# WU-CVGL/CasualHDRSplat

Hardware: AMD Instinct MI355X
Metric: train-step images/sec (fwd+bwd raster) @ 1M Gaussians 1080p (higher is better)
Workload: dtype f32; 1 GPU; c3: 1000000 Gaussians, 1920x1080, SH degree 3, HDR radiance + CRF tone-map, 1 pose(s)/view, 1 view(s)/step (one per GPU); num_rendered_R=6777809, R_prime=3025699, pixel_pair_evals_E=559372855, seed=0, binning=sync-free fixed capacity 1.25*R, launch=eager (one enqueue per kernel)

## Files before the change

### casualhdrsplat_amd/csrc/render.hip

```cpp
#include "hs_common.h"

namespace hs {

namespace {

constexpr float kAlphaMin = 1.0f / 255.0f;
constexpr float kAlphaMax = 0.99f;
constexpr float kTmin = 0.0001f;
constexpr float kLogEps = 1e-8f;


enum {
    kStBwdTrips = 0,
    kStBwdEmpty = 1,
    kStBwdActivePix = 2,
    kStBwdCulled = 3,
    kStBwdHist = 4,
    kStBwdStaged = 10,
    kStBwdBatches = 11,
    kStFwdTrips = 12, kStFwdEmpty = 13, kStFwdActivePix = 14, kStFwdCulled = 15, kStFwdStaged = 16, kStFwdBatches = 17,
    kStCount = 24
};
struct WaveStats {
    unsigned long long v[kStCount];
// ... 473 lines not shown
    float sumH = 0.f, sumL = 0.f;
    const float* planes = pose_hdr + (int64_t)f * N * 3 * HW + j;
    for (int k = 0; k < N; ++k) {
        const float Hv = planes[(int64_t)k * 3 * HW];
        sumH += Hv;
        if (hdr && !(flags & HS_FLAG_BLUR_HDR)) sumL += crf_eval(crf, ch, Hv);
    }
    const float inv = 1.f / (float)N;
    const float meanH = sumH * inv;
    pose_hdr[((int64_t)F * N + f) * 3 * HW + j] = meanH;
    if (hdr) {
        if (out_hdr) out_hdr[i] = meanH;
        out_color[i] = (flags & HS_FLAG_BLUR_HDR) ? crf_eval(crf, ch, meanH) : sumL * inv;
    } else {
        out_color[i] = meanH;
    }
}

__global__ void __launch_bounds__(1024) order_tiles_kernel(int nb, int gx, int n_static, const uint32_t* work,
                                                           uint32_t* order) {
    constexpr int kBins = 1024, kT = 1024;
    __shared__ uint32_t s_hist[kBins];
    __shared__ uint32_t s_scan[kT / 64];
    __shared__ uint32_t s_thr_bin, s_thr_take;
    const int x = blockIdx.x, t = threadIdx.x;
    const int per = nb / 8, rem = nb % 8;
    const int cnt = per + (x < rem ? 1 : 0);
    const int n_keep = n_static > x ? (n_static - x + 7) / 8 : 0;
    const int n_light = cnt - n_keep;
    int q_base = 0;
    for (int y = 0; y < x; ++y) q_base += (per + (y < rem ? 1 : 0)) - (n_static > y ? (n_static - y + 7) / 8 : 0);
    const int E = (cnt + kT - 1) / kT;
    const int k0 = t * E, k1 = min(cnt, (t + 1) * E);
    if (E > 64) {
        for (int k = k0; k < k1; ++k) order[x + 8 * k] = (uint32_t)xcd_strip_tile(x + 8 * k, nb, gx);
        return;
    }
    auto block_excl_scan = [&](uint32_t v, uint32_t* total) -> uint32_t {
        uint32_t incl = v;
#pragma unroll
        for (int d = 1; d < 64; d <<= 1) { const uint32_t u = __shfl_up(incl, d); if ((t & 63) >= d) incl += u; }
        __syncthreads();
        if ((t & 63) == 63) s_scan[t >> 6] = incl;
        __syncthreads();
        uint32_t add = 0, tot = 0;
        for (int w = 0; w < kT / 64; ++w) { const uint32_t c = s_scan[w]; if (w < (t >> 6)) add += c; tot += c; }
        *total = tot;
        return add + incl - v;
    };
    auto bin_of = [&](int k) { return (int)min((uint32_t)(kBins - 1), work[xcd_strip_tile(x + 8 * k, nb, gx)] >> 1); };
    s_hist[t] = 0;
    if (t == 0) { s_thr_bin = 0; s_thr_take = 0; }
    __syncthreads();
    for (int k = k0; k < k1; ++k) atomicAdd(&s_hist[bin_of(k)], 1u);
    __syncthreads();
    {
        uint32_t tot;
        const uint32_t h = s_hist[t];
        const uint32_t below = block_excl_scan(h, &tot);
        if (below < (uint32_t)n_light && below + h >= (uint32_t)n_light) { s_thr_bin = t; s_thr_take = (uint32_t)n_light - below; }
    }
    __syncthreads();
    const int thr = (int)s_thr_bin;
    const uint32_t take = s_thr_take;
    uint32_t in_thr = 0;
    for (int k = k0; k < k1; ++k) in_thr += bin_of(k) == thr ? 1u : 0u;
    uint32_t tot_thr;
    uint32_t thr_rank = block_excl_scan(in_thr, &tot_thr);
    uint64_t light_mask = 0;
    uint32_t kept = 0;
    for (int k = k0; k < k1; ++k) {
        const int b = bin_of(k);
        const bool light = n_light > 0 && (b < thr || (b == thr && thr_rank++ < take));
        light_mask |= (uint64_t)light << (k - k0);
        kept += !light;
    }
    uint32_t tot_kept;
    uint32_t kpos = block_excl_scan(kept, &tot_kept);
    uint32_t qpos = (uint32_t)k0 - kpos;
    for (int k = k0; k < k1; ++k) {
        const uint32_t vt = (uint32_t)xcd_strip_tile(x + 8 * k, nb, gx);
        if ((light_mask >> (k - k0)) & 1ull) order[n_static + q_base + (int)qpos++] = vt;
        else order[x + 8 * (int)kpos++] = vt;
    }
}

constexpr int kCrfPixPerWave = 1024;

struct CrfGradArgs {
    int64_t HW; int N, F, flags;
    const float* pose_hdr; Crf crf; const float* exposure; const float* dL_dcolor; float* partials;
    int bx, planes;
};

template <int NW, int NH = 1>
__device__ __forceinline__ void crf_grad_body(const CrfGradArgs& A, const int bxi, const int plane_in,
                                              unsigned long long* const s_tab64) {
    static_assert(NH == 1 || NW == 1, "pieces in turn: one-wave workgroups only");
    constexpr int NP = NW * NH;
    static_assert(NP == 2 || NP == 4, "the pieces' float sums are added in a stated order");
    const int64_t HW = A.HW; const int N = A.N, flags = A.flags; const float* pose_hdr = A.pose_hdr; Crf crf = A.crf;
    const float* exposure = A.exposure; const float* dL_dcolor = A.dL_dcolor; float* partials = A.partials;
    int* const s_tab32 = reinterpret_cast<int*>(s_tab64);
    __shared__ float s_wave[NP][4];
    __shared__ float s_max[NW];
    const int K = crf.K;
    for (int i = threadIdx.x; i < K - 1; i += NW * 64) s_tab64[i] = 0ull;
    const bool blur_hdr = (flags & HS_FLAG_BLUR_HDR) && N > 1;
    const float gs = blur_hdr ? 1.f : 1.f / (float)N;
    const float scale = (float)(K - 1) / (crf.umax - crf.umin);
    const int plane = plane_in;
    const int pose = plane / 3, ch = plane - 3 * pose;
    const int frame = blur_hdr ? pose : (A.F > 1 ? pose / N : 0);
    crf.dt = exposure[frame];
    const float* Hp = pose_hdr + ((int64_t)(blur_hdr ? A.F * N + frame : pose) * 3 + ch) * HW;
    const float* gp = dL_dcolor + ((int64_t)frame * 3 + ch) * HW;
    const float* t = crf.table + ch * K;
    const int lane = threadIdx.x & 63, wave = threadIdx.x >> 6;

    float Hv[NH][16], g[NH][16];
#pragma unroll
    for (int h = 0; h < NH; ++h) {
        const int64_t i16 = ((int64_t)bxi * (NP * 64) + h * 64 + threadIdx.x) * 16;
        if (i16 + 16 <= HW && (HW & 3) == 0) {
#pragma unroll
            for (int q = 0; q < 4; ++q) {
                const float4 h4 = reinterpret_cast<const float4*>(Hp + i16)[q];
                const float4 g4 = reinterpret_cast<const float4*>(gp + i16)[q];
                Hv[h][4 * q] = h4.x; Hv[h][4 * q + 1] = h4.y; Hv[h][4 * q + 2] = h4.z; Hv[h][4 * q + 3] = h4.w;
                g[h][4 * q] = g4.x * gs; g[h][4 * q + 1] = g4.y * gs; g[h][4 * q + 2] = g4.z * gs; g[h][4 * q + 3] = g4.w * gs;
            }
        } else {
#pragma unroll
            for (int e = 0; e < 16; ++e) {
                const bool ok = i16 + e < HW;
                Hv[h][e] = ok ? Hp[i16 + e] : 0.f;
                g[h][e] = ok ? gp[i16 + e] * gs : 0.f;
            }
        }
    }
    float mx = 0.f;
#pragma unroll
    for (int h = 0; h < NH; ++h)
#pragma unroll
        for (int e = 0; e < 16; ++e) mx = fmaxf(mx, fabsf(g[h][e]));
#pragma unroll
    for (int d = 32; d >= 1; d >>= 1) mx = fmaxf(mx, __shfl_xor(mx, d));
    if (lane == 0) s_max[wave] = mx;
    __syncthreads();
    mx = s_max[0];
    if constexpr (NW >= 2) mx = fmaxf(mx, s_max[1 % NW]);
    if constexpr (NW == 4) mx = fmaxf(mx, fmaxf(s_max[2 % NW], s_max[3 % NW]));
    int xexp = 0;
    if (mx > 0.f && mx < 3.0e38f) (void)frexpf(mx, &xexp);
    const float to_fix = ldexpf(1.f, 19 - xexp), from_fix = ldexpf(1.f, xexp - 19);

#pragma unroll
    for (int h = 0; h < NH; ++h) {
        float gexp = 0.f, g_lo = 0.f, g_hi = 0.f;
        int run = -1;
        float r0 = 0.f, r1 = 0.f;
        auto flush = [&]() {
            atomicAdd(&s_tab32[2 * run], __float2int_rn(r0 * to_fix));
            atomicAdd(&s_tab32[2 * run + 1], __float2int_rn(r1 * to_fix));
        };
#pragma unroll
        for (int e = 0; e < 16; ++e) {
            int idx; float f, xv; bool in;
            crf_locate(crf, Hv[h][e], idx, f, xv, in);
            const bool lo = idx == 0 && f == 0.f, hi = idx == K - 2 && f == 1.f;
            g_lo += lo ? g[h][e] : 0.f;
            g_hi += hi ? g[h][e] : 0.f;
            if (!lo && !hi) {
                if (idx != run) {
                    if (run >= 0) flush();
                    run = idx; r0 = 0.f; r1 = 0.f;
                }
                r0 += (1.f - f) * g[h][e];
                r1 += f * g[h][e];
            }
            if (in) gexp += g[h][e] * (t[idx + 1] - t[idx]) * scale * __builtin_amdgcn_rcpf(xv) * Hv[h][e];
        }
        if (run >= 0) flush();
        gexp = wave_sum_hi(gexp);
        g_lo = wave_sum_hi(g_lo);
        g_hi = wave_sum_hi(g_hi);
        if (lane == 63) { s_wave[wave + h][0] = gexp; s_wave[wave + h][1] = g_lo; s_wave[wave + h][2] = g_hi; }
    }
    __syncthreads();
    auto pieces = [&](int c) {
        float v = s_wave[0][c] + s_wave[1][c];
        if constexpr (NP == 4) v = (v + s_wave[2 % NP][c]) + s_wave[3 % NP][c];
        return v;
    };
    float* dst = partials + ((int64_t)plane_in * A.bx + bxi) * (K + 1);
    for (int k = threadIdx.x; k <= K; k += NW * 64) {
        float v;
        if (k == K) {
            v = pieces(0);
        } else {
            long long acc = 0;
            if (k < K - 1) acc += (long long)s_tab32[2 * k];
            if (k > 0) acc += (long long)s_tab32[2 * (k - 1) + 1];
            v = (float)acc * from_fix;
            if (k == 0) v += pieces(1);
            if (k == K - 1) v += pieces(2);
        }
        dst[k] = v;
    }
}

struct RenderBwd {
    int W, H, gx, gy, ntiles, N, F, flags;
    const uint2* ranges; const uint32_t* point_list; const float4* rec; const float* bg;
    const float* final_T; const uint32_t* n_contrib; const float* pose_hdr;
    const float* dL_dcolor; const float* dL_dhdr; const float* dL_dalpha; const float* dL_dinvdepth;
    float4* pair_grads;
    uint8_t* pair_flags;
    const uint8_t* pair_act;
    Crf crf;
    const float* exposure;
    unsigned long long* stats;
    unsigned long long* timeline;
    uint32_t* queue;
    const uint32_t* tile_order;
    int grid_tiles;
    CrfGradArgs crf_tail;
};

__device__ __forceinline__ float pixel_grad(const RenderBwd& p, const Crf& c, int pose, int frame, int ch, int64_t pix, int64_t HW) {
    const float invN = 1.f / (float)p.N;
    const int64_t gpl = ((int64_t)frame * 3 + ch) * HW + pix;
    float g = p.dL_dcolor[gpl];
    if (!(p.flags & HS_FLAG_HDR)) return g * invN;
    float out = 0.f;
    if (p.N == 1 || !(p.flags & HS_FLAG_BLUR_HDR)) {
        const float Hv = p.pose_hdr[((int64_t)pose * 3 + ch) * HW + pix];
        out = crf_grad_H(c, ch, Hv, g * invN);
    } else {
        const float Hm = p.pose_hdr[((int64_t)(p.F * p.N + frame) * 3 + ch) * HW + pix];
        out = crf_grad_H(c, ch, Hm, g) * invN;
    }
    if (p.dL_dhdr) out += p.dL_dhdr[gpl] * invN;
    return out;
}

struct PixB {
    float T, dL0, dL1, dL2, q;
    float dLd;
    uint32_t last;
};

__device__ __forceinline__ void load_pixel_bwd(const RenderBwd& p, PixB& s, bool inside, int pose, int frame, int px, int py) {
    const int64_t HW = (int64_t)p.H * p.W;
    const int64_t pix = (int64_t)py * p.W + px;
    s.T = 0.f; s.dL0 = s.dL1 = s.dL2 = 0.f; s.last = 0;
    if (inside) {
        s.T = p.final_T[(int64_t)pose * HW + pix];
        s.last = p.n_contrib[(int64_t)pose * HW + pix];
        Crf c = p.crf;
        if (p.flags & HS_FLAG_HDR) c.dt = p.exposure[frame];
        s.dL0 = pixel_grad(p, c, pose, frame, 0, pix, HW);
        s.dL1 = pixel_grad(p, c, pose, frame, 1, pix, HW);
        s.dL2 = pixel_grad(p, c, pose, frame, 2, pix, HW);
    }
    float bg_dot = (p.bg[0] * s.dL0 + p.bg[1] * s.dL1) + p.bg[2] * s.dL2;
    if (p.dL_dalpha && inside) bg_dot -= p.dL_dalpha[pix] / (float)p.N;
    s.q = bg_dot;
    s.dLd = (p.dL_dinvdepth && inside) ? p.dL_dinvdepth[pix] / (float)p.N : 0.f;
}

struct PairB {
    f2 T, q, dL0, dL1, dL2, dLd;
};
__device__ __forceinline__ f2 splat(float v) { f2 r = {v, v}; return r; }
__device__ __forceinline__ PairB pack_pair(const PixB& a, const PixB& b) {
    PairB s;
    s.T = f2{a.T, b.T}; s.q = f2{a.q, b.q};
    s.dL0 = f2{a.dL0, b.dL0}; s.dL1 = f2{a.dL1, b.dL1}; s.dL2 = f2{a.dL2, b.dL2};
    s.dLd = f2{a.dLd, b.dLd};
    return s;
}
template <bool DEPTH>
__device__ __forceinline__ void step_bwd_pair(PairB& s, bool act0, bool act1, f2 G, f2 alpha, float o, float r, float g,
                                              float b, float invd, f2& sw, f2& dop, f2& dch) {
    const f2 ae = {act0 ? alpha.x : 0.f, act1 ? alpha.y : 0.f};
    const f2 one_m = splat(1.f) - ae;
    const f2 rcp = {__builtin_amdgcn_rcpf(one_m.x), __builtin_amdgcn_rcpf(one_m.y)};
    s.T *= rcp;
    dch = ae * s.T;
    f2 cd = (splat(r) * s.dL0 + pk_mul_hi(f2{r, g}, s.dL1)) + splat(b) * s.dL2;
    if constexpr (DEPTH) cd += splat(invd) * s.dLd;
    const f2 diff = cd - s.q;
    const f2 gd = G * (diff * s.T);
    s.q += ae * diff;
    dop = f2{act0 ? gd.x : 0.f, act1 ? gd.y : 0.f};
    sw = splat(o) * dop;
}

constexpr int kTailPct = 8;
constexpr int kAccF = 12;
constexpr int kBwdWave = 64;
#ifndef HS_TUNE_BWD_KB
#define HS_TUNE_BWD_KB 48
#endif
#ifndef HS_TUNE_BWD_WAVES
#define HS_TUNE_BWD_WAVES 4
#endif
constexpr int kBwdKB = HS_TUNE_BWD_KB;
constexpr int bwd_stage_floats(int ent_f) { return (kBwdKB + 1) * ent_f > 7 * 256 ? (kBwdKB + 1) * ent_f : 7 * 256; }

__device__ __forceinline__ void lane_pixels4(int lane, int sx, int sy, int& px, int& py0) {
    const int blk = lane >> 4;
    px = sx + 8 * (blk & 1) + (lane & 7);
    py0 = sy + 8 * (blk >> 1) + 4 * ((lane >> 3) & 1);
}

template <bool DEPTH, bool STATS>
__global__ void __launch_bounds__(kBwdWave) __attribute__((amdgpu_waves_per_eu((DEPTH || STATS) ? 1 : HS_TUNE_BWD_WAVES)))
render_bwd_kernel(RenderBwd p) {
    constexpr int KB = kBwdKB;
    constexpr int NV = DEPTH ? 10 : 9;
    constexpr int kEntF = kAccF + 4 * NV;
    constexpr int kEntB = kEntF * 4;
    static_assert(kEntB % 16 == 0, "LDS entry records must stay 16-byte aligned");
    static_assert(KB <= kBwdWave, "one staged entry per lane, one ballot per list");
    constexpr int kSentinel = KB * kEntB;
    constexpr int kListLen = KB + 8;
    constexpr int kStageF = bwd_stage_floats(kEntF);
    __shared__ __attribute__((aligned(16))) float s_ent[kStageF];
    __shared__ uint16_t s_list[4][kListLen];

    const int lane = threadIdx.x;
    if constexpr (!STATS) {
        if ((int)blockIdx.x >= p.grid_tiles) {
            const int qd = (int)blockIdx.x - p.grid_tiles;
            crf_grad_body<1, 2>(p.crf_tail, qd % p.crf_tail.bx, qd / p.crf_tail.bx, reinterpret_cast<unsigned long long*>(s_ent));
            return;
        }
    }
    const int n_tail = (int)((int64_t)p.grid_tiles * kTailPct / 100);
    const int n_static = p.grid_tiles - n_tail;
    for (;;) {
    int bidx = blockIdx.x;
    if ((int)blockIdx.x >= n_static) {
        uint32_t q = 0;
        if (lane == 0) {
            q = atomicAdd(p.queue, 1u);
            if (q == 2u * (uint32_t)n_tail - 1u) atomicExch(p.queue, 0u);
        }
        q = __builtin_amdgcn_readfirstlane(q);
        if (q >= (uint32_t)n_tail) return;
        bidx = n_static + (int)q;
    }
    const int vt = p.tile_order ? (int)p.tile_order[bidx] : xcd_strip_tile(bidx, p.grid_tiles, p.gx);
    const int pose = vt / p.ntiles;
    const int tile = vt - pose * p.ntiles;
    const int tx = tile % p.gx, ty = tile / p.gx;
    const int blk = lane >> 4;
    const int plane = 2 * (blk & 1) + (blk >> 1);
    const int sx = tx * kTile, sy = ty * kTile;
    int px, py0;
    lane_pixels4(lane, sx, sy, px, py0);
    const float pxf = (float)px;
    const f2 pyfA = {(float)py0, (float)(py0 + 1)}, pyfB = {(float)(py0 + 2), (float)(py0 + 3)};

    unsigned long long t_start = 0;
    if constexpr (STATS) t_start = wall_clock64();
    const uint2 range = p.ranges[vt];

    PairB psA, psB;
    uint32_t last0, last1, last2, last3;
    {
        __syncthreads();
        const int qc = lane & 15, qr = lane >> 4;
        const int frame = p.F > 1 ? pose / p.N : 0;
        float* const o = s_ent;
#pragma unroll
        for (int k = 0; k < 4; ++k) {
            const int row = qr + 4 * k;
            PixB t;
            load_pixel_bwd(p, t, sx + qc < p.W && sy + row < p.H, pose, frame, sx + qc, sy + row);
            const int r = row * 16 + qc;
            o[r] = t.T; o[256 + r] = t.dL0; o[512 + r] = t.dL1; o[768 + r] = t.dL2; o[1024 + r] = t.q;
            o[1280 + r] = t.dLd; o[1536 + r] = __uint_as_float(t.last);
        }
        __syncthreads();
        const float* const m = o + (py0 - sy) * 16 + (px - sx);
        psA.T = f2{m[0], m[16]};                  psB.T = f2{m[32], m[48]};
        psA.dL0 = f2{m[256], m[256 + 16]};        psB.dL0 = f2{m[256 + 32], m[256 + 48]};
        psA.dL1 = f2{m[512], m[512 + 16]};        psB.dL1 = f2{m[512 + 32], m[512 + 48]};
        psA.dL2 = f2{m[768], m[768 + 16]};        psB.dL2 = f2{m[768 + 32], m[768 + 48]};
        psA.q = f2{m[1024], m[1024 + 16]};        psB.q = f2{m[1024 + 32], m[1024 + 48]};
        psA.dLd = f2{m[1280], m[1280 + 16]};      psB.dLd = f2{m[1280 + 32], m[1280 + 48]};
        last0 = __float_as_uint(m[1536]); last1 = __float_as_uint(m[1536 + 16]);
        last2 = __float_as_uint(m[1536 + 32]); last3 = __float_as_uint(m[1536 + 48]);
        __syncthreads();
        if (lane < kAccF) s_ent[KB * kEntF + lane] = 0.f;
    }

    const int n_proc = (int)__builtin_amdgcn_readfirstlane(wave_max_u32(max(max(last0, last1), max(last2, last3))));

    int red_off = -1;
    const int red_j = lane & 3;
    {
        const int k = (lane & 15) >> 2;
        if (red_j == 0) red_off = k;
        else if (red_j == 1) red_off = 4 + k;
        else if (red_j == 2 && k == 0) red_off = 8;
        else if (DEPTH && red_j == 2 && k == 1) red_off = 9;
        if (red_off >= 0) red_off = (kAccF + NV * plane + red_off) * 4;
    }
    char* const ent = reinterpret_cast<char*>(s_ent);
    float* const my_ent = s_ent + lane * kEntF;
    const uint16_t* const my_list = s_list[blk];
    WaveStats ws;
    if constexpr (STATS) ws.clear();
    const int nb = (n_proc + KB - 1) / KB;
    uint32_t id_next = 0, act_next = 0;
    if (nb > 0) {
        const int base = (nb - 1) * KB;
        if (lane < n_proc - base) {
            id_next = p.point_list[range.x + base + lane];
            act_next = p.pair_act[(int64_t)range.x + base + lane];
        }
    }
    for (int bi = nb - 1; bi >= 0; --bi) {
        const int base = bi * KB;
        const int cnt = min(KB, n_proc - base);
        if constexpr (STATS) { ws.v[kStBwdStaged] += cnt; ws.v[kStBwdBatches] += 1; }
        __syncthreads();
        const uint32_t act = lane < cnt ? act_next : 0u;
        const bool taken = act != 0;
        if (taken) {
            const float4* r = p.rec + kRecF4 * (int64_t)id_next;
            float4 ra = r[0], rb = r[1];
            float4 rc = r[2];
            if constexpr (DEPTH) rc.y = 1.f / rc.y;
            scale_entry(ra, rb);
            reinterpret_cast<float4*>(my_ent)[0] = ra;
            reinterpret_cast<float4*>(my_ent)[1] = rb;
            reinterpret_cast<float4*>(my_ent)[2] = rc;
        }
        if (bi > 0 && lane < KB) {
            id_next = p.point_list[range.x + base - KB + lane];
            act_next = p.pair_act[(int64_t)range.x + base - KB + lane];
        }
        {
            int maxn = 0;
            [[maybe_unused]] int n_half[2] = {0, 0};
#pragma unroll
            for (int b = 0; b < 4; ++b) {
                const uint32_t gbit = 1u << (2 * (b & 1) + (b >> 1));
                uint16_t* lst = s_list[b];
                const uint64_t m = __ballot((act & gbit) != 0);
                const int c = __popcll(m);
                if ((m >> lane) & 1ull) lst[c - 1 - mask_prefix(m)] = (uint16_t)(lane * kEntB);
#pragma unroll
                for (int t = lane; t < kListLen; t += 64)
                    if (t >= c) lst[t] = (uint16_t)kSentinel;
                maxn = max(maxn, c);
                n_half[b >> 1] = max(n_half[b >> 1], c);
            }
            if constexpr (STATS) ws.v[kStBwdCulled] += (uint32_t)cnt - (uint32_t)__popcll(__ballot(taken));
            __syncthreads();
            const int lim0 = ((int)last0 - base) * kEntB, lim1 = ((int)last1 - base) * kEntB;
            const int lim2 = ((int)last2 - base) * kEntB, lim3 = ((int)last3 - base) * kEntB;
            int jb = (int)my_list[0];
            const int n_it = __builtin_amdgcn_readfirstlane(maxn);
            for (int ti = 0; ti < n_it; ++ti) {
                int jn = (int)my_list[ti + 1];
                asm("" : "+v"(jn));
                const float4 a = *reinterpret_cast<const float4*>(ent + jb);
                const float4 b = *reinterpret_cast<const float4*>(ent + jb + 16);
                const float2 c = *reinterpret_cast<const float2*>(ent + jb + 32);
                const float cb = c.x;
                const float invd = DEPTH ? c.y : 0.f;
                const float dx = a.x - pxf;
                const f2 dyA = a.y - pyfA, dyB = a.y - pyfB;
                const float t = a.z * dx * dx, u = a.w * dx;
                const f2 pwA = dyA * (b.x * dyA + u) + t, pwB = dyB * (b.x * dyB + u) + t;
                const float G0 = hs_exp2(pwA.x), G1 = hs_exp2(pwA.y), G2 = hs_exp2(pwB.x), G3 = hs_exp2(pwB.y);
                const float al0 = fminf(kAlphaMax, b.y * G0), al1 = fminf(kAlphaMax, b.y * G1);
                const float al2 = fminf(kAlphaMax, b.y * G2), al3 = fminf(kAlphaMax, b.y * G3);
                const bool act0 = (jb < lim0) && (pwA.x <= 0.f) && (al0 >= kAlphaMin);
                const bool act1 = (jb < lim1) && (pwA.y <= 0.f) && (al1 >= kAlphaMin);
                const bool act2 = (jb < lim2) && (pwB.x <= 0.f) && (al2 >= kAlphaMin);
                const bool act3 = (jb < lim3) && (pwB.y <= 0.f) && (al3 >= kAlphaMin);
                if constexpr (STATS) {
                    const uint64_t lanes = __ballot(act0 || act1 || act2 || act3);
#pragma unroll
                    for (int h = 0; h < 2; ++h) {
                        if (ti < n_half[h]) {
                            const int nl = __popc((uint32_t)(lanes >> (32 * h)));
                            ws.v[kStBwdTrips] += 1;
                            ws.v[kStBwdEmpty] += nl == 0;
                            const int bin = nl == 0 ? 0 : nl <= 4 ? 1 : nl <= 8 ? 2 : nl <= 16 ? 3 : nl <= 32 ? 4 : 5;
                            ws.v[kStBwdHist + bin] += 1;
                        }
                    }
                    ws.v[kStBwdActivePix] += __popcll(__ballot(act0)) + __popcll(__ballot(act1)) + __popcll(__ballot(act2)) +
                                             __popcll(__ballot(act3));
                }
                f2 swA, dopA, dchA, swB, dopB, dchB;
                step_bwd_pair<DEPTH>(psA, act0, act1, f2{G0, G1}, f2{al0, al1}, b.y, b.z, b.w, cb, invd, swA, dopA, dchA);
                step_bwd_pair<DEPTH>(psB, act2, act3, f2{G2, G3}, f2{al2, al3}, b.y, b.z, b.w, cb, invd, swB, dopB, dchB);
                const f2 sw = swA + swB;
                const f2 mA = swA * dyA, mB = swB * dyB;
                const f2 m = mA + mB;
                const f2 m2 = mA * dyA + mB * dyB;
                const f2 c0 = dchA * psA.dL0 + dchB * psB.dL0;
                const f2 c1 = dchA * psA.dL1 + dchB * psB.dL1;
                const f2 c2 = dchA * psA.dL2 + dchB * psB.dL2;
                float g[9];
                g[0] = (sw.x + sw.y) * dx;
                g[1] = m.x + m.y;
                g[2] = g[0] * dx;
                g[3] = g[1] * dx;
                g[4] = m2.x + m2.y;
                g[5] = (dopA.x + dopA.y) + (dopB.x + dopB.y);
                g[6] = c0.x + c0.y;
                g[7] = c1.x + c1.y;
                g[8] = c2.x + c2.y;
                float g9 = 0.f;
                if constexpr (DEPTH) {
                    const f2 cd = dchA * psA.dLd + dchB * psB.dLd;
                    g9 = cd.x + cd.y;
                }
                float t0, t1, t2;
                row_reduce<DEPTH>(g, g9, t0, t1, t2);
                if (red_off >= 0) *reinterpret_cast<float*>(ent + jb + red_off) = red_j == 0 ? t0 : red_j == 1 ? t1 : t2;
                jb = jn;
            }
        }
        __syncthreads();
        if (taken) {
            float v[10] = {0.f, 0.f, 0.f, 0.f, 0.f, 0.f, 0.f, 0.f, 0.f, 0.f};
#pragma unroll
            for (int pl = 0; pl < 4; ++pl) {
                const bool on = (act >> pl) & 1u;
#pragma unroll
                for (int q = 0; q < NV; ++q) {
                    const float x = my_ent[kAccF + NV * pl + q];
                    v[q] += on ? x : 0.f;
                }
            }
            const float4 a = reinterpret_cast<const float4*>(my_ent)[0];
            const float4 c = reinterpret_cast<const float4*>(my_ent)[2];
            const float A = a.z * (-2.f / kLog2e), B = a.w * (-1.f / kLog2e), C = my_ent[4] * (-2.f / kLog2e);
            const float ddelx_dx = 0.5f * (float)p.W, ddely_dy = 0.5f * (float)p.H;
            const float gmx = -(A * v[0] + B * v[1]) * ddelx_dx;
            const float gmy = -(C * v[1] + B * v[0]) * ddely_dy;
            const int rad = __float_as_int(c.z);
            const uint32_t off = __float_as_uint(c.w);
            const int rminx = min(p.gx, max(0, (int)((a.x - (float)rad) / (float)kTile)));
            const int rminy = min(p.gy, max(0, (int)((a.y - (float)rad) / (float)kTile)));
            const int rmaxx = min(p.gx, max(0, (int)((a.x + (float)rad + (float)(kTile - 1)) / (float)kTile)));
            const int64_t slot = (int64_t)off + (int64_t)(ty - rminy) * (rmaxx - rminx) + (tx - rminx);
            p.pair_flags[slot] = 1;
            float4* o = p.pair_grads + kPairF4 * slot;
            o[0] = make_float4(gmx, gmy, -0.5f * v[2], -v[3]);
            o[1] = make_float4(-0.5f * v[4], v[5], v[6], v[7]);
            float zero = 0.f;
            asm volatile("" : "+v"(zero));
            o[2] = make_float4(v[8], v[9], zero, zero);
            if constexpr (kPairF4 == 4) o[3] = make_float4(zero, zero, zero, zero);
        }
    }
    if constexpr (STATS) {
        ws.flush(p.stats);
        if (p.timeline && lane == 0) {
            p.timeline[3 * bidx + 0] = t_start;
            p.timeline[3 * bidx + 1] = wall_clock64();
            const uint32_t xcc = __builtin_amdgcn_s_getreg((3 << 11) | (0 << 6) | 20);
            const uint32_t hw = __builtin_amdgcn_s_getreg((31 << 11) | (0 << 6) | 4);
            p.timeline[3 * bidx + 2] = ((unsigned long long)xcc << 32) | hw;
        }
    }
    if ((int)blockIdx.x < n_static) return;
    }
}

__global__ void __launch_bounds__(256) crf_grad_kernel(CrfGradArgs A) {
    extern __shared__ unsigned long long s_crf_tab[];
    crf_grad_body<4>(A, (int)blockIdx.x, (int)blockIdx.y, s_crf_tab);
}

__global__ void __launch_bounds__(256) crf_reduce_kernel(CrfReduce c) { crf_reduce_block(c, (int)blockIdx.x); }

}

static bool orders_tiles(int grid) { return grid <= 6 * 3072; }


int launch_render_fwd(const hs_fwd_args& a, const hs_layout& L, hipStream_t s, unsigned long long* stats) {
    const hs_dims& d = a.dims;
    RenderFwd p;
    p.W = d.W; p.H = d.H; p.gx = (d.W + kTile - 1) / kTile;
    const int gy = (d.H + kTile - 1) / kTile;
    const int F = frames_of(d);
    p.ntiles = p.gx * gy; p.N = d.n_poses / F; p.flags = a.flags;
    char* bin = (char*)a.binning; char* img = (char*)a.image; char* geom = (char*)a.geom;
    p.ranges = (const uint2*)(bin + L.ranges); p.point_list = (const uint32_t*)(bin + L.point_list);
    p.rec = (const float4*)(geom + L.rec); p.bg = a.bg;
    p.out_color = a.out_color; p.out_hdr = a.out_hdr;
    p.final_T = (float*)(img + L.final_T); p.n_contrib = (uint32_t*)(img + L.n_contrib);
    const bool need_pose = (a.flags & HS_FLAG_HDR) || p.N > 1;
    p.pose_hdr = need_pose ? (float*)(img + L.pose_hdr) : nullptr;
    p.crf.table = a.crf_table; p.crf.K = a.crf_K; p.crf.umin = a.crf_umin; p.crf.umax = a.crf_umax; p.crf.dt = 1.f;
    p.exposure = a.exposure;
    p.out_invdepth = a.out_invdepth;
    p.stats = stats; p.timeline = nullptr;
    p.pair_act = (uint8_t*)bin + L.pair_act;
    p.tile_work = (uint32_t*)(img + L.tile_work);
    const int grid = p.ntiles * d.n_poses;
    if (stats) {
        if (a.out_invdepth) render_fwd_kernel<true, true><<<grid, kBatch, 0, s>>>(p);
        else render_fwd_kernel<false, true><<<grid, kBatch, 0, s>>>(p);
    } else if (a.out_invdepth) render_fwd_kernel<true, false><<<grid, kBatch, 0, s>>>(p);
    else render_fwd_kernel<false, false><<<grid, kBatch, 0, s>>>(p);
    HS_LAUNCH_CHECK();
    if (orders_tiles(grid)) {
        const int n_static = grid - (int)((int64_t)grid * kTailPct / 100);
        order_tiles_kernel<<<8, 1024, 0, s>>>(grid, p.gx, n_static, p.tile_work, (uint32_t*)(img + L.tile_order));
        HS_LAUNCH_CHECK();
    }
    if (p.N > 1) {
        const int64_t HW = (int64_t)d.W * d.H;
        resolve_kernel<<<ceil_div((int64_t)F * 3 * HW, 256), 256, 0, s>>>(HW, p.N, F, a.flags, p.pose_hdr, p.crf, a.exposure,
                                                                         a.out_color, a.out_hdr);
        HS_LAUNCH_CHECK();
    }
    return HS_OK;
}

static bool crf_grad_args(const hs_bwd_args& a, const hs_layout& L, CrfGradArgs& A, int waves = 4) {
    const hs_dims& d = a.dims;
    if (!((a.flags & HS_FLAG_HDR) && (a.dL_dcrf_table || a.dL_dexposure))) return false;
    A.crf.table = a.crf_table; A.crf.K = a.crf_K; A.crf.umin = a.crf_umin; A.crf.umax = a.crf_umax; A.crf.dt = 1.f;
    A.HW = (int64_t)d.W * d.H; A.F = frames_of(d); A.N = d.n_poses / A.F; A.flags = a.flags;
    A.partials = (float*)((char*)a.bwd + L.crf_partials);
    A.pose_hdr = (const float*)((const char*)a.image + L.pose_hdr);
    A.exposure = a.exposure; A.dL_dcolor = a.dL_dout_color;
    const bool blur_hdr = (a.flags & HS_FLAG_BLUR_HDR) && A.N > 1;
    A.planes = 3 * (blur_hdr ? A.F : d.n_poses);
    A.bx = ceil_div(A.HW, (int64_t)waves * kCrfPixPerWave);
    return true;
}

int launch_crf_bwd(const hs_bwd_args& a, const hs_layout& L, hipStream_t s, CrfReduce* defer, bool in_render_tail) {
    CrfGradArgs A;
    if (!crf_grad_args(a, L, A, in_render_tail ? 2 : 4)) return HS_OK;
    if (!in_render_tail)
        crf_grad_kernel<<<dim3(A.bx, A.planes), 256, (size_t)(a.crf_K - 1) * sizeof(unsigned long long), s>>>(A);
    CrfReduce cr;
    cr.partials = A.partials; cr.bx = A.bx; cr.planes = A.planes; cr.K = a.crf_K; cr.d_table = a.dL_dcrf_table;
    cr.F = A.F;
    cr.d_exposure = a.dL_dexposure; cr.nblocks = ceil_div(3 * a.crf_K + cr.F, 4);
    if (defer) *defer = cr;
    else crf_reduce_kernel<<<cr.nblocks, 256, 0, s>>>(cr);
    HS_LAUNCH_CHECK();
    return HS_OK;
}

int launch_render_bwd(const hs_bwd_args& a, const hs_layout& L, hipStream_t s, unsigned long long* stats,
                      unsigned long long* timeline, bool crf_in_tail) {
    const hs_dims& d = a.dims;
    RenderBwd p;
    p.W = d.W; p.H = d.H; p.gx = (d.W + kTile - 1) / kTile; p.gy = (d.H + kTile - 1) / kTile;
    p.F = frames_of(d);
    p.ntiles = p.gx * p.gy; p.N = d.n_poses / p.F; p.flags = a.flags;
    const char* bin = (const char*)a.binning; const char* img = (const char*)a.image; const char* geom = (const char*)a.geom;
    p.ranges = (const uint2*)(bin + L.ranges); p.point_list = (const uint32_t*)(bin + L.point_list);
    p.rec = (const float4*)(geom + L.rec); p.bg = a.bg;
    p.final_T = (const float*)(img + L.final_T); p.n_contrib = (const uint32_t*)(img + L.n_contrib);
    p.pose_hdr = (const float*)(img + L.pose_hdr);
    p.dL_dcolor = a.dL_dout_color; p.dL_dhdr = a.dL_dout_hdr; p.dL_dalpha = a.dL_dout_alpha;
    p.dL_dinvdepth = a.dL_dout_invdepth;
    p.pair_grads = (float4*)((char*)a.bwd + L.pair_grads);
    p.crf.table = a.crf_table; p.crf.K = a.crf_K; p.crf.umin = a.crf_umin; p.crf.umax = a.crf_umax; p.crf.dt = 1.f;
    p.exposure = a.exposure;
    p.pair_flags = (uint8_t*)a.binning + L.pair_flags;
    p.pair_act = (const uint8_t*)a.binning + L.pair_act;
    p.stats = stats; p.timeline = timeline;
    p.queue = &((hs_counters*)((char*)a.geom + L.counters))->reserved[3];
    p.tile_order = orders_tiles(p.ntiles * d.n_poses) ? (const uint32_t*)(img + L.tile_order) : nullptr;
    int grid = p.ntiles * d.n_poses;
    p.grid_tiles = grid;
    if (crf_in_tail && !stats && crf_grad_args(a, L, p.crf_tail, 2)) grid += p.crf_tail.bx * p.crf_tail.planes;
    if (stats) {
        if (a.dL_dout_invdepth) render_bwd_kernel<true, true><<<grid, kBwdWave, 0, s>>>(p);
        else render_bwd_kernel<false, true><<<grid, kBwdWave, 0, s>>>(p);
    } else if (a.dL_dout_invdepth) render_bwd_kernel<true, false><<<grid, kBwdWave, 0, s>>>(p);
    else render_bwd_kernel<false, false><<<grid, kBwdWave, 0, s>>>(p);
    HS_LAUNCH_CHECK();
    return HS_OK;
}

int render_stats_count() { return kStCount; }

int render_bwd_tail_max_knots() { return bwd_stage_floats(kAccF + 4 * 9) / 2 + 1; }

int64_t crf_partial_floats(int K, int64_t HW, int n_poses) {
    return K > 0 ? (int64_t)ceil_div(HW, 2 * kCrfPixPerWave) * 3 * n_poses * (K + 1) : 0;
}

}
```

Measured before the change: 983.5 images/s.

## Compact active bwd entries per batch and pool per-plane reduction slots

The backward raster kernel now scans a 128-entry window of the point list, compacts only entries with nonzero pair activity into a batch of up to KB takers, and stores per-plane gradient partials in a shared slot pool sized by actual plane hits. Before, each entry reserved fixed space for all four planes. This is meant to skip staging and iterating over inactive entries and to use LDS better, so KB can rise from 48 to 64. In exchange it adds extra ballots, a compaction pass through LDS, and count-based thresholds for each pixel's last index, which makes the indexing more complex.

Result: no change. 993.2 images/s (median of 6 runs) (+1.0%).

```diff
diff --git a/casualhdrsplat_amd/csrc/render.hip b/casualhdrsplat_amd/csrc/render.hip
--- a/casualhdrsplat_amd/csrc/render.hip
+++ b/casualhdrsplat_amd/csrc/render.hip
@@ -799,13 +799,20 @@
 constexpr int kAccF = 12;
 constexpr int kBwdWave = 64;
 #ifndef HS_TUNE_BWD_KB
-#define HS_TUNE_BWD_KB 48
+#define HS_TUNE_BWD_KB 64
+#endif
+#ifndef HS_TUNE_BWD_POOL
+#define HS_TUNE_BWD_POOL 160
 #endif
 #ifndef HS_TUNE_BWD_WAVES
 #define HS_TUNE_BWD_WAVES 4
 #endif
 constexpr int kBwdKB = HS_TUNE_BWD_KB;
-constexpr int bwd_stage_floats(int ent_f) { return (kBwdKB + 1) * ent_f > 7 * 256 ? (kBwdKB + 1) * ent_f : 7 * 256; }
+constexpr int kBwdPool = HS_TUNE_BWD_POOL;
+constexpr int kBwdWin = 128;
+constexpr int bwd_stage_floats(int nv) {
+    return (kBwdKB + 1) * kAccF + (kBwdPool + 1) * nv > 7 * 256 ? (kBwdKB + 1) * kAccF + (kBwdPool + 1) * nv : 7 * 256;
+}
 
 __device__ __forceinline__ void lane_pixels4(int lane, int sx, int sy, int& px, int& py0) {
     const int blk = lane >> 4;
@@ -817,16 +824,27 @@
 __global__ void __launch_bounds__(kBwdWave) __attribute__((amdgpu_waves_per_eu((DEPTH || STATS) ? 1 : HS_TUNE_BWD_WAVES)))
 render_bwd_kernel(RenderBwd p) {
     constexpr int KB = kBwdKB;
+    constexpr int POOL = kBwdPool;
+    constexpr int WIN = kBwdWin;
     constexpr int NV = DEPTH ? 10 : 9;
-    constexpr int kEntF = kAccF + 4 * NV;
+    constexpr int kEntF = kAccF;
     constexpr int kEntB = kEntF * 4;
+    constexpr int kSlotB = NV * 4;
     static_assert(kEntB % 16 == 0, "LDS entry records must stay 16-byte aligned");
-    static_assert(KB <= kBwdWave, "one staged entry per lane, one ballot per list");
+    static_assert(KB >= 1 && KB <= kBwdWave, "one taker per lane, one ballot per list");
+    static_assert(POOL >= 4 && POOL <= 255, "a taker needs up to four slots");
     constexpr int kSentinel = KB * kEntB;
+    constexpr int kPoolB = (KB + 1) * kEntB;
+    constexpr int kSpareB = kPoolB + POOL * kSlotB;
     constexpr int kListLen = KB + 8;
-    constexpr int kStageF = bwd_stage_floats(kEntF);
+    constexpr int kCompB = kPoolB, kCountB = kPoolB + KB * 8;
+    static_assert(KB * 8 + WIN + 4 <= (POOL + 1) * kSlotB, "the compaction borrows the pool");
+    static_assert(kSpareB + kSlotB <= 65535, "list items are 16-bit byte offsets");
+    constexpr int kStageF = bwd_stage_floats(NV);
+    static_assert(kStageF * 4 >= kSpareB + kSlotB, "records, pool and spare slot fit the staging area");
     __shared__ __attribute__((aligned(16))) float s_ent[kStageF];
     __shared__ uint16_t s_list[4][kListLen];
+    __shared__ uint16_t s_slot[4][kListLen];
 
     const int lane = threadIdx.x;
     if constexpr (!STATS) {
@@ -855,7 +873,6 @@
     const int tile = vt - pose * p.ntiles;
     const int tx = tile % p.gx, ty = tile / p.gx;
     const int blk = lane >> 4;
-    const int plane = 2 * (blk & 1) + (blk >> 1);
     const int sx = tx * kTile, sy = ty * kTile;
     int px, py0;
     lane_pixels4(lane, sx, sy, px, py0);
@@ -906,31 +923,75 @@
         else if (red_j == 1) red_off = 4 + k;
         else if (red_j == 2 && k == 0) red_off = 8;
         else if (DEPTH && red_j == 2 && k == 1) red_off = 9;
-        if (red_off >= 0) red_off = (kAccF + NV * plane + red_off) * 4;
+        if (red_off >= 0) red_off *= 4;
     }
     char* const ent = reinterpret_cast<char*>(s_ent);
     float* const my_ent = s_ent + lane * kEntF;
     const uint16_t* const my_list = s_list[blk];
+    const uint16_t* const my_slot = s_slot[blk];
     WaveStats ws;
     if constexpr (STATS) ws.clear();
-    const int nb = (n_proc + KB - 1) / KB;
-    uint32_t id_next = 0, act_next = 0;
-    if (nb > 0) {
-        const int base = (nb - 1) * KB;
-        if (lane < n_proc - base) {
-            id_next = p.point_list[range.x + base + lane];
-            act_next = p.pair_act[(int64_t)range.x + base + lane];
-        }
-    }
-    for (int bi = nb - 1; bi >= 0; --bi) {
-        const int base = bi * KB;
-        const int cnt = min(KB, n_proc - base);
-        if constexpr (STATS) { ws.v[kStBwdStaged] += cnt; ws.v[kStBwdBatches] += 1; }
+    int cur = n_proc;
+    uint32_t id_n0 = 0, id_n1 = 0, act_n0 = 0, act_n1 = 0;
+    auto prefetch = [&]() {
+        const int64_t top = (int64_t)range.x + cur - 1 - lane;
+        act_n0 = 0; act_n1 = 0;
+        if (lane < cur) { id_n0 = p.point_list[top]; act_n0 = p.pair_act[top]; }
+        if (lane + 64 < cur) { id_n1 = p.point_list[top - 64]; act_n1 = p.pair_act[top - 64]; }
+    };
+    prefetch();
+    while (cur > 0) {
+        const uint32_t a0 = act_n0 & 0xFu, a1 = act_n1 & 0xFu;
+        const uint32_t id0 = id_n0, id1 = id_n1;
+        const uint64_t tm0 = __ballot(a0 != 0), tm1 = __ballot(a1 != 0);
+        const int tk0 = mask_prefix(tm0), tk1 = __popcll(tm0) + mask_prefix(tm1);
+        int pp0 = __popc(a0), pp1 = __popc(a1);
+#pragma unroll
+        for (int b = 0; b < 4; ++b) {
+            const uint64_t m0 = __ballot((a0 >> b) & 1u), m1 = __ballot((a1 >> b) & 1u);
+            pp0 += mask_prefix(m0);
+            pp1 += __popcll(m0) + mask_prefix(m1);
+        }
+        const bool ok0 = tk0 + (a0 != 0) <= KB && pp0 <= POOL;
+        const bool ok1 = tk1 + (a1 != 0) <= KB && pp1 <= POOL;
+        const int run = min(cur, __popcll(__ballot(ok0)) + __popcll(__ballot(ok1)));
+        const bool in0 = lane < run && a0 != 0, in1 = lane + 64 < run && a1 != 0;
+        const int ntk = __popcll(__ballot(in0)) + __popcll(__ballot(in1));
+        const int top = cur;
+        cur -= run;
         __syncthreads();
-        const uint32_t act = lane < cnt ? act_next : 0u;
-        const bool taken = act != 0;
+        if (ntk > 0) {
+            uint2* const comp = reinterpret_cast<uint2*>(ent + kCompB);
+            uint8_t* const count = reinterpret_cast<uint8_t*>(ent + kCountB);
+            if (in0) comp[tk0] = make_uint2(id0, a0);
+            if (in1) comp[tk1] = make_uint2(id1, a1);
+            count[lane] = (uint8_t)tk0;
+            count[64 + lane] = (uint8_t)tk1;
+            if (lane == 0) count[WIN] = (uint8_t)(__popcll(tm0) + __popcll(tm1));
+        }
+        prefetch();
+        if (ntk == 0) {
+            if constexpr (STATS) ws.v[kStBwdCulled] += (uint32_t)run;
+            continue;
+        }
+        if constexpr (STATS) { ws.v[kStBwdStaged] += ntk; ws.v[kStBwdBatches] += 1; ws.v[kStBwdCulled] += (uint32_t)(run - ntk); }
+        __syncthreads();
+        const bool taken = lane < ntk;
+        uint32_t act = 0, id_mine = 0;
         if (taken) {
-            const float4* r = p.rec + kRecF4 * (int64_t)id_next;
+            const uint2 ia = reinterpret_cast<const uint2*>(ent + kCompB)[lane];
+            id_mine = ia.x; act = ia.y;
+        }
+        int thr0, thr1, thr2, thr3;
+        {
+            const uint8_t* const count = reinterpret_cast<const uint8_t*>(ent + kCountB);
+            thr0 = (int)count[min(max(top - (int)last0, 0), run)] * kEntB;
+            thr1 = (int)count[min(max(top - (int)last1, 0), run)] * kEntB;
+            thr2 = (int)count[min(max(top - (int)last2, 0), run)] * kEntB;
+            thr3 = (int)count[min(max(top - (int)last3, 0), run)] * kEntB;
+        }
+        if (taken) {
+            const float4* r = p.rec + kRecF4 * (int64_t)id_mine;
             float4 ra = r[0], rb = r[1];
             float4 rc = r[2];
             if constexpr (DEPTH) rc.y = 1.f / rc.y;
@@ -939,35 +1000,38 @@
             reinterpret_cast<float4*>(my_ent)[1] = rb;
             reinterpret_cast<float4*>(my_ent)[2] = rc;
         }
-        if (bi > 0 && lane < KB) {
-            id_next = p.point_list[range.x + base - KB + lane];
-            act_next = p.pair_act[(int64_t)range.x + base - KB + lane];
-        }
+        uint64_t gmask[4];
+        int goff[4];
         {
-            int maxn = 0;
+            int maxn = 0, off = 0;
             [[maybe_unused]] int n_half[2] = {0, 0};
 #pragma unroll
             for (int b = 0; b < 4; ++b) {
                 const uint32_t gbit = 1u << (2 * (b & 1) + (b >> 1));
                 uint16_t* lst = s_list[b];
+                uint16_t* slt = s_slot[b];
                 const uint64_t m = __ballot((act & gbit) != 0);
                 const int c = __popcll(m);
-                if ((m >> lane) & 1ull) lst[c - 1 - mask_prefix(m)] = (uint16_t)(lane * kEntB);
+                if ((m >> lane) & 1ull) {
+                    const int t = mask_prefix(m);
+                    lst[t] = (uint16_t)(lane * kEntB);
+                    slt[t] = (uint16_t)(kPoolB + (off + t) * kSlotB);
+                }
 #pragma unroll
                 for (int t = lane; t < kListLen; t += 64)
-                    if (t >= c) lst[t] = (uint16_t)kSentinel;
+                    if (t >= c) { lst[t] = (uint16_t)kSentinel; slt[t] = (uint16_t)kSpareB; }
+                gmask[b] = m; goff[b] = off;
+                off += c;
                 maxn = max(maxn, c);
                 n_half[b >> 1] = max(n_half[b >> 1], c);
             }
-            if constexpr (STATS) ws.v[kStBwdCulled] += (uint32_t)cnt - (uint32_t)__popcll(__ballot(taken));
             __syncthreads();
-            const int lim0 = ((int)last0 - base) * kEntB, lim1 = ((int)last1 - base) * kEntB;
-            const int lim2 = ((int)last2 - base) * kEntB, lim3 = ((int)last3 - base) * kEntB;
             int jb = (int)my_list[0];
             const int n_it = __builtin_amdgcn_readfirstlane(maxn);
             for (int ti = 0; ti < n_it; ++ti) {
                 int jn = (int)my_list[ti + 1];
                 asm("" : "+v"(jn));
+                const int sb = (int)my_slot[ti];
                 const float4 a = *reinterpret_cast<const float4*>(ent + jb);
                 const float4 b = *reinterpret_cast<const float4*>(ent + jb + 16);
                 const float2 c = *reinterpret_cast<const float2*>(ent + jb + 32);
@@ -980,10 +1044,10 @@
                 const float G0 = hs_exp2(pwA.x), G1 = hs_exp2(pwA.y), G2 = hs_exp2(pwB.x), G3 = hs_exp2(pwB.y);
                 const float al0 = fminf(kAlphaMax, b.y * G0), al1 = fminf(kAlphaMax, b.y * G1);
                 const float al2 = fminf(kAlphaMax, b.y * G2), al3 = fminf(kAlphaMax, b.y * G3);
-                const bool act0 = (jb < lim0) && (pwA.x <= 0.f) && (al0 >= kAlphaMin);
-                const bool act1 = (jb < lim1) && (pwA.y <= 0.f) && (al1 >= kAlphaMin);
-                const bool act2 = (jb < lim2) && (pwB.x <= 0.f) && (al2 >= kAlphaMin);
-                const bool act3 = (jb < lim3) && (pwB.y <= 0.f) && (al3 >= kAlphaMin);
+                const bool act0 = (jb >= thr0) && (pwA.x <= 0.f) && (al0 >= kAlphaMin);
+                const bool act1 = (jb >= thr1) && (pwA.y <= 0.f) && (al1 >= kAlphaMin);
+                const bool act2 = (jb >= thr2) && (pwB.x <= 0.f) && (al2 >= kAlphaMin);
+                const bool act3 = (jb >= thr3) && (pwB.y <= 0.f) && (al3 >= kAlphaMin);
                 if constexpr (STATS) {
                     const uint64_t lanes = __ballot(act0 || act1 || act2 || act3);
 #pragma unroll
@@ -1026,7 +1090,7 @@
                 }
                 float t0, t1, t2;
                 row_reduce<DEPTH>(g, g9, t0, t1, t2);
-                if (red_off >= 0) *reinterpret_cast<float*>(ent + jb + red_off) = red_j == 0 ? t0 : red_j == 1 ? t1 : t2;
+                if (red_off >= 0) *reinterpret_cast<float*>(ent + sb + red_off) = red_j == 0 ? t0 : red_j == 1 ? t1 : t2;
                 jb = jn;
             }
         }
@@ -1035,10 +1099,13 @@
             float v[10] = {0.f, 0.f, 0.f, 0.f, 0.f, 0.f, 0.f, 0.f, 0.f, 0.f};
 #pragma unroll
             for (int pl = 0; pl < 4; ++pl) {
+                const int b = ((pl & 1) << 1) | (pl >> 1);
                 const bool on = (act >> pl) & 1u;
+                const int so = on ? kPoolB + (goff[b] + mask_prefix(gmask[b])) * kSlotB : kSpareB;
+                const float* const slot = reinterpret_cast<const float*>(ent + so);
 #pragma unroll
                 for (int q = 0; q < NV; ++q) {
-                    const float x = my_ent[kAccF + NV * pl + q];
+                    const float x = slot[q];
                     v[q] += on ? x : 0.f;
                 }
             }
@@ -1196,7 +1263,7 @@
 
 int render_stats_count() { return kStCount; }
 
-int render_bwd_tail_max_knots() { return bwd_stage_floats(kAccF + 4 * 9) / 2 + 1; }
+int render_bwd_tail_max_knots() { return bwd_stage_floats(9) / 2 + 1; }
 
 int64_t crf_partial_floats(int K, int64_t HW, int n_poses) {
     return K > 0 ? (int64_t)ceil_div(HW, 2 * kCrfPixPerWave) * 3 * n_poses * (K + 1) : 0;
```
